# bluescarni/heyoka

Hardware: AMD Instinct MI355X
Metric: ODE systems x steps/sec (fp64) (higher is better)
Workload: dtype f64

## Files before the change

heyoka_amd/csrc/hip_emit_cluster2.cpp:

```cpp
#include <algorithm>
#include <cstdio>
#include <functional>

#include "hip_emit_cluster2_gen.hpp"
#include "logging.hpp"

namespace heyoka_amd::cluster2_detail
{

cluster2_gen::cluster2_gen(const taylor_program &p_, const emit_options &opts_, std::string &why_not_, bool allow_one_lane_,
                           std::uint32_t min_lanes_)
    : c2_emit(p_, opts_.order), p(p_), opts(opts_), why_not(why_not_), allow_one_lane(allow_one_lane_), min_lanes(min_lanes_),
      n_eq(p_.n_eq), order(opts_.order)
{
    std::string s = opts.dev.v5_opts;
    std::replace(s.begin(), s.end(), '+', ',');
    for (std::size_t b = 0, en = 0; b <= s.size(); b = en + 1u) {
        en = std::min(s.find(',', b), s.size());
        v5_flags.insert(s.substr(b, en - b));
    }
}

cluster2_attempt cluster2_gen::run()
{
// ... 1515 lines not shown
                    if (have == want && pe_lane_ev.count(cl) == 0u) {
                        pe_lane_ev[cl] = {static_cast<std::uint32_t>(ev), pe.c};
                        pe_lane_sign[cl] = pe.sign;
                        ev_on_lane[ev] = 1;
                        break;
                    }
                }
            }
        }
        const bool ev_ok = emit_event_jets_inline(*opts.ev_prog, opts, sv, ev_store, ev_code, ev_coeffs, why_ev,
                                                  use_lanes ? &hooks : nullptr, &ev_on_lane);
        if (!ev_ok) {
            pe_lane_ev.clear();
        }
        if (ev_ok) {
            ev_inline = true;
            const auto pick = [&](const std::vector<std::uint64_t> &v) {
                std::string r = std::to_string(v[0]) + "u";
                for (std::size_t c = v.size(); c-- > 1u;) {
                    r = "(l == " + std::to_string(c) + "u ? " + std::to_string(v[c]) + "u : " + r + ")";
                }
                return r;
            };
            for (std::size_t pp = 0; use_lanes && pp < hooks.leaf_vars.size(); ++pp) {
                std::vector<std::uint64_t> off, str_, zoff, zstr;
                for (const auto var : hooks.leaf_vars[pp]) {
                    const auto &lc = loc[var];
                    const auto &src_ = lc.derived ? loc[lc.parent] : lc;
                    off.push_back(src_.off);
                    str_.push_back(src_.stride);
                    zoff.push_back(lc.off);
                    zstr.push_back(lc.stride);
                }
                src << "const unsigned evo" << pp << " = " << pick(off) << " + q * " << pick(str_) << ";\n";
                if (hooks.leaf_class[pp] == 1) {
                    src << "const unsigned evz" << pp << " = " << pick(zoff) << " + q * " << pick(zstr) << ";\n";
                }
            }
            if (!pe_lane_ev.empty()) {
                std::string on = "0.0", cst = "0.0", row = std::to_string(opts.ev_prog->ev_u.size()) + "u";
                for (const auto &[lane_, evc] : pe_lane_ev) {
                    const auto ls = "(l == " + std::to_string(lane_) + "u ? ";
                    on = ls + (pe_lane_sign.at(lane_) < 0 ? "-1.0 : " : "1.0 : ") + on + ")";
                    cst = ls + fp_literal(evc.second) + " : " + cst + ")";
                    row = ls + std::to_string(evc.first) + "u : " + row + ")";
                }
                src << "const double pe_on = " << on << ";\nconst double pe_c = " << cst << ";\nconst u64 pe_row = (u64)" << row
                    << " * " << (order + 1u) << "u;\n";
            }
        }
    }
}

void cluster2_gen::text_pickup()
{
    src << R"HIP(
// Work distribution. Propagation (steps per system differ): a device-side queue, one group of systems at a time (taking
// wavefronts, which is what lets the partial-line accesses to the SoA arrays meet in L2). Single steps (equal cost per
// group): a static interleaved schedule - group = iteration * wavefronts + wavefront - with the same locality and no
const u64 hy_waves = (u64)gridDim.x * HY_WPB;
const bool hy_static = (HY_MODE != 1) && (HY_NO_STATIC == 0);
u64 hy_it = 0;
bool hy_queue_empty = false;
for (;;) {
u64 base = 0;
if (hy_static) {
    // (Exit decided per workgroup: the cooperative store of the Taylor coefficients below has workgroup barriers. A
    // wavefront beyond the end of the ensemble in a live workgroup replicates the last system, without side effects.)
    if (HY_M4 && (hy_it * (u64)gridDim.x + blockIdx.x) * (HY_WPB * SPW) >= N) break;
    base = (hy_it * hy_waves + gwave) * SPW;
    ++hy_it;
} else {
    if (lane == 0u) base = atomicAdd((u64 *)(a.counters + 2), (u64)SPW);
}
// NOTE: through readfirstlane the position is a scalar for the compiler and the exit of the work loop a wave-uniform
// branch (a shuffle / the wavefront index leave it "divergent": exec-mask bookkeeping around the whole step loop).
base = ((u64)__builtin_amdgcn_readfirstlane((unsigned)(base >> 32)) << 32) | (u64)__builtin_amdgcn_readfirstlane((unsigned)base);
if (!(HY_M4 && hy_static) && base >= N) break;
// NOTE: lanes beyond the end of the ensemble replicate the last system (no side effects).
bool live = (base + q) < N;
u64 s = live ? (base + q) : (N - 1u);
double t_hi = a.time_hi[s], t_lo = a.time_lo[s];
)HIP";
    for (std::uint32_t i = 0; i < p.n_par; ++i) {
        src << "const double par_" << i << " = a.pars[(u64)" << i << "u * N + s];\n";
    }
    for (const auto t : lane_par_tbls) {
        src << "const double lp" << t << " = a.pars[(u64)" << utname(t) << " * N + s];\n";
    }
    for_each_owner([&](auto &, auto &ow) {
        src << row0_w(ow) << " = a.state[(u64)hy_utbl[" << ow.var_tbl * L << "u + l] * N + s];\n";
    });
    src << "HY_WSYNC();\n" << (jet_lds ? "" : "__builtin_amdgcn_fence(__ATOMIC_SEQ_CST, \"wavefront\");\n");
    src << R"HIP(
hy_df tfin, rem;
tfin.hi = 0.0; tfin.lo = 0.0; rem.hi = 0.0; rem.lo = 0.0;
bool t_dir = true;
double mdt = __builtin_inf();
double step_lim = 0.0;
double thr = 0.0;
if (HY_MODE == 1) {
    tfin.hi = (a.tfin_hi != nullptr) ? a.tfin_hi[s] : a.tfin_s_hi;
    tfin.lo = (a.tfin_hi != nullptr) ? a.tfin_lo[s] : a.tfin_s_lo;
    hy_df tcur; tcur.hi = t_hi; tcur.lo = t_lo;
    rem = hy_df_sub(tfin, tcur);
    t_dir = (rem.hi > 0.0) || (rem.hi == 0.0 && rem.lo >= 0.0);
    if (a.lim != nullptr) mdt = a.lim[s];
    // (Propagation from grid point to grid point - hy_kargs::pad bit 2 in mode 1, emitted_module::grid_multi_step: the
    // system leaves the step loop after the first step which reaches a.tc_thr[s], with the coefficients of that step stored.)
    if ((a.pad & 4) != 0) thr = a.tc_thr[s];
} else {
    step_lim = a.lim[s];
    // (Taylor coefficients of a lock-step sweep on demand - hy_kargs::pad bit 2, the loop of propagate_grid() without a
    // callback: the NEXT GRID TIME of every system - a.tc_thr, or a.tfin_hi for callers of before round 6 -, and only the
    // steps which reach it store their coefficients - see emitted_module::tc_by_threshold.)
    if ((a.pad & 4) != 0) thr = (a.tc_thr != nullptr) ? a.tc_thr[s] : a.tfin_hi[s];
}
u64 n_steps = 0, iter = 0;
double min_h = __builtin_inf(), max_h = 0.0, last_h = 0.0;
i64 outcome = HY_OC_SUCCESS;
// NOTE: the step loop is left by the whole wavefront at once (wave-uniform exit): a system which has reached its final
// time keeps executing steps of length zero with all its bookkeeping frozen by selects (fin) until the other
// systems of the wavefront are done - a wavefront executes an iteration as long as one of its lanes is active
// anyway. With a per-lane exit the loop-carried values of the lanes which have left live across several
// hundred live registers of the remaining ones, which is where this toolchain's live-range splitting goes
// wrong (DESIGN.md, toolchain notes).
bool fin = false;
// (Did the system leave the step loop through a step clamped to its remaining time? hy_kargs::grid_done.)
bool gfin = false;
int nf_seen = 0;
// (Stepper with events which evaluates the event equations itself: does this system need its Taylor coefficients in
// memory? See "On-demand Taylor coefficients" below. hy_kargs::pad: bit 0 = store them for every system, bit 1 = store
// NOTHING but them - the regeneration launch on the snapshot of the state before the step.)
bool need_tc = true;
const bool hy_tc_only = HY_M4 && ((a.pad & 2) != 0);
)HIP";
    bk_lds = one_lane;
    if (bk_lds) {
        bk_store();
        src << "HY_WSYNC();\n";
    }
    src << "for (;;) {\n";
    src << body;
}

void cluster2_gen::text_selector()
{
    if (!pe_lane_ev.empty()) {
        src << "HY_WSYNC();\n";
        std::string dK[3];
        for (std::uint32_t i = 0; i < 3u; ++i) {
            src << "const double pe_d" << i << " = " << slabk(order, utname(st1.s[i][0])) << " - " << slabk(order, utname(st1.s[i][1]))
                << ";\n";
            dK[i] = "pe_d" + std::to_string(i);
        }
        for (std::uint32_t i = 0; i < 3u; ++i) {
            src << "double pe_q" << i << " = " << dK[i] << " * " << sD[i][0] << ";\n";
            for (std::uint32_t j = 1; 2u * j < order; ++j) {
                src << "pe_q" << i << " = __builtin_fma(" << sD[i][j] << ", " << sD[i][order - j] << ", pe_q" << i << ");\n";
            }
            if (order % 2u == 0u) {
                src << "pe_q" << i << " = __builtin_fma(0.5 * " << sD[i][order / 2u] << ", " << sD[i][order / 2u] << ", pe_q" << i
                    << ");\n";
            }
        }
        src << "const double pe_bh = (pe_q0 + pe_q1) + pe_q2;\n";
        pe_g.resize(order + 1u);
        src << "const double pe_b0s = " << sB[0] << " * pe_on;\n";
        src << "const double pe_g0 = pe_b0s + pe_c;\n";
        pe_g[0] = "pe_g0";
        for (std::uint32_t k = 1; k < order; ++k) {
            src << "const double pe_g" << k << " = " << sB[k] << " * pe_b0s;\n";
            pe_g[k] = "pe_g" + std::to_string(k);
        }
        src << "const double pe_g" << order << " = (pe_bh + pe_bh) * pe_on;\n";
        pe_g[order] = "pe_g" + std::to_string(order);
        src << "m0 = hy_nmax(m0, fabs(pe_g0));\nmo = hy_nmax(mo, fabs(pe_g" << order
            << "));\nmom1 = hy_nmax(mom1, fabs(pe_g" << order - 1u << "));\n";
    }

    const bool packed_tail = L >= 4u;
    const auto red_ex = [&](std::uint32_t m, const char *v) -> std::string {
        if (m == 1u) {
            return std::string("hy_dpp<0xB1>(") + v + ")";
        }
        if (m == 2u) {
            return std::string("hy_dpp<0x4E>(") + v + ")";
        }
        if (m == 4u && L % 16u == 0u) {
// ... 48 lines not shown
        for (const auto &o2 : gr.owners) {
            if (o2.derived && o2.parent == ow.col) {
                dv = &o2;
            }
        }
        tail_passes.push_back({&ow, dv, dv != nullptr && pk_tbl.count(ow.col) != 0u, {}, {}});
    });
    kstride = static_cast<std::uint64_t>(spw) * n_colp;
    if (one_lane && !m4 && jet_lds && opts.high_accuracy && packed_tail && !v5_flag("notailrd")) {
        src << "// (Jet reads of the final evaluation issued ahead of the selector.)\n";
        const auto hoist = [&](const std::string &ex) {
            auto nm = "trd" + std::to_string(n_trd++);
            src << "const double " << nm << " = " << ex << ";\n";
            return nm;
        };
        for (auto &tp : tail_passes) {
            const auto cs = std::to_string(tp.ow->col);
            if (tp.packed) {
                const auto &tb = pk_tbl.at(tp.ow->col);
                if (!lane_sum) {
                    src << "const double *const pk_jh" << cs << " = jetw + q * " << jet_sys(*tp.ow) << "u + hy_utbl[" << tb[1] * L << "u + l];\n";
                    src << "const double *const pk_fh" << cs << " = lds_fac + hy_utbl[" << tb[2] * L << "u + l];\n";
                }
                tp.rows.resize(order + 1u);
                tp.facs.resize(order + 1u);
                for (std::uint32_t k = 1; k <= order; ++k) {
                    tp.rows[k] = hoist("pk_jh" + cs + "[" + std::to_string((k - 1u) * kstride) + "]");
                    tp.facs[k] = hoist("pk_fh" + cs + "[" + std::to_string(k) + "]");
                }
            } else {
                for (std::uint32_t k = 0; k <= order; ++k) {
                    tp.rows.push_back(hoist("jr" + cs + "[" + std::to_string(k * kstride) + "]"));
                }
            }
        }
        src << "__builtin_amdgcn_sched_barrier(0);\n";
    }
    if (packed_tail) {
        src << "const double nw = (hy_q0 & (nv <= 1.0)) ? 1.0 : nv;\n";
        src << "const double lg = " << (sel_scalar ? "hy_sel_log_s" : "hy_sel_log") << "(nw);\n";
        src << "const double lg0 = hy_dpp<0x00>(lg), lg1 = hy_dpp<0x55>(lg), lg2 = hy_dpp<0xAA>(lg);\n";
        src << "const double lr_o = (lg0 - lg1) * " << fp_literal(1. / static_cast<double>(order)) << ";\n";
        src << "const double lr_om1 = (lg0 - lg2) * " << fp_literal(1. / static_cast<double>(order - 1u)) << ";\n";
        src << "const double rho_m = " << (sel_scalar ? "hy_sel_exp_s" : "exp") << "(hy_min(lr_o, lr_om1));\n";
    } else {
        src << "const double num_rho = (m0 <= 1.0) ? 1.0 : m0;\n";
        src << "const double lr_o = log(num_rho / mo) * " << fp_literal(1. / static_cast<double>(order)) << ";\n";
        src << "const double lr_om1 = log(num_rho / mom1) * " << fp_literal(1. / static_cast<double>(order - 1u)) << ";\n";
        src << "const double rho_m = exp(hy_min(lr_o, lr_om1));\n";
    }
    if (bk_lds) {
        bk_load();
    }
    src << R"HIP(
double lim;
if (HY_MODE == 1) {
    hy_df m; m.lo = 0.0;
    // NOTE: selects, not an if/else on the (per-lane) direction: see the note on HY_LIBM1.
    m.hi = t_dir ? mdt : -mdt;
    const bool lt_fwd = hy_df_lt(rem, m), lt_bwd = hy_df_lt(m, rem);
    const bool rem_first = (t_dir & lt_fwd) | (!t_dir & lt_bwd);
    lim = rem_first ? rem.hi : m.hi;
} else {
    lim = step_lim;
}
lim = fin ? 0.0 : lim;
)HIP";
    src << "double h = rho_m * " << fp_literal(rhofac(order)) << ";\n";
    src << "h = hy_min(h, fabs(lim));\nh = (lim < 0.0) ? -h : h;\n";
    src << "h = fin ? 0.0 : h;\n";
}

void cluster2_gen::text_event_exclusion()
{
    if (ev_inline) {
        src << "bool maybe0 = false, pe_m0 = false;\n{\nconst double ah = fabs(h);\n";
        for (const auto &c : ev_coeffs) {
            if (c.empty()) {
                continue;
            }
            src << "{\ndouble r = fabs(" << c[order] << ");\n";
            for (std::uint32_t k = order - 1u; k >= 1u; --k) {
                src << "r = r * ah + fabs(" << c[k] << ");\n";
            }
            src << "r = r * ah;\nmaybe0 = maybe0 | !(fabs(" << c[0] << ") > r * 1.00000001);\n}\n";
        }
        if (!pe_g.empty()) {
            src << "{\ndouble r = fabs(" << pe_g[order] << ");\n";
            for (std::uint32_t k = order - 1u; k >= 1u; --k) {
                src << "r = r * ah + fabs(" << pe_g[k] << ");\n";
            }
            src << "r = r * ah;\npe_m0 = (pe_on != 0.0) & !(fabs(" << pe_g[0] << ") > r * 1.00000001);\n}\n";
        }
        src << "}\nneed_tc = ((a.pad & 1) != 0);\nbool ev_possible = false;\n";
        const auto sys_any = [&](const char *v) {
            return "(((__builtin_amdgcn_ballot_w64(" + std::string(v) + ") >> ((threadIdx.x & 63u) & " + std::to_string(64u - L) + "u)) & "
                   + std::to_string((std::uint64_t(1) << L) - 1u) + "ull) != 0ull)";
        };
        src << "if (__builtin_amdgcn_ballot_w64(maybe0 | pe_m0) != 0ull) {\n";
        src << "bool maybe = false, maybe_te = false;\nconst double lo_h = (h < 0.0) ? h : 0.0, hi_h = (h < 0.0) ? 0.0 : h;\n";
        const auto enclosure = [&](const std::vector<std::string> &c) {
            src << "{\ndouble lo = " << c[order] << ", hi = lo, mm = fabs(lo);\n";
            for (std::uint32_t i = 1; i <= order; ++i) {
                src << "{\nconst double p0 = lo * lo_h, p1 = lo * hi_h, p2 = hi * lo_h, p3 = hi * hi_h;\n"
                    << "const double mn = fmin(fmin(p0, p1), fmin(p2, p3)), mx = fmax(fmax(p0, p1), fmax(p2, p3));\n"
                    << "lo = mn + " << c[order - i] << ";\nhi = mx + " << c[order - i] << ";\n"
                    << "mm = fmax(mm, fmax(fabs(lo), fabs(hi)));\n}\n";
            }
        };
        for (std::size_t ci = 0; ci < ev_coeffs.size(); ++ci) {
            const auto &c = ev_coeffs[ci];
            if (c.empty()) {
                continue;
            }
            enclosure(c);
            src << "const bool excl = (((lo > 0.0) & (hi > 0.0)) | ((lo < 0.0) & (hi < 0.0))) & (fmin(fabs(lo), fabs(hi)) > 1e-8 * mm);\n"
                << "maybe = maybe | !excl;\n" << (ci < opts.n_t_events ? "maybe_te = maybe_te | !excl;\n" : "") << "}\n";
        }
        src << "bool pe_m = false;\n";
        if (!pe_g.empty()) {
// ... 103 lines not shown
                    }
                }
            }
        }
        src << xn << " = res;\n";
        if (dv != nullptr) {
            src << xd << " = resd;\n";
        }
        src << "}\n";
        const auto new_at = [&](const owner_slot &o) {
            return ev_inline ? ("slab[" + std::to_string(o.col * L) + "u + l]") : row0_w(o);
        };
        upd.emplace_back(xn, row0_r(ow), new_at(ow));
        if (dv != nullptr) {
            upd.emplace_back(xd, row0_r(*dv), new_at(*dv));
        }
    }
    if (n_trd_used != n_trd) {
        throw std::logic_error("hy_taylor (one lane per pair): " + std::to_string(n_trd - n_trd_used)
                               + " jet reads of the final evaluation were issued ahead of the selector and not consumed");
    }
    for (std::uint32_t c = 0; !one_lane && c < n_hslots; ++c) {
        upd.emplace_back("xn" + std::to_string(c), "hc" + std::to_string(c) + "[0]", "hc" + std::to_string(c) + "[0]");
        if (m4) {
            src << "const double xn" << c << " = hc" << c << "[0];\n";
            continue;
        }
        src << "double xn" << c << ";\n{\nconst double *c = hc" << c << ";\n";
        if (opts.high_accuracy) {
            src << "double res = c[0], comp = 0.0, cur_h = h;\n#pragma unroll\n";
            src << "for (unsigned k = 1; k <= " << order << "u; ++k) {\n";
            src << "const double tmp = c[(u64)k * " << kstride << "u] * cur_h;\nconst double y = tmp - comp;\n";
            src << "const double t = res + y;\ncomp = (t - res) - y;\nres = t;\ncur_h = cur_h * h;\n}\n";
        } else {
            src << "double res = c[(u64)" << order << "u * " << kstride << "u];\n#pragma unroll\n";
            src << "for (unsigned k = 1; k <= " << order << "u; ++k) {\n";
            src << "res = c[(u64)(" << order << "u - k) * " << kstride << "u] + res * h;\n}\n";
        }
        src << "xn" << c << " = res;\n}\n";
    }
    src << R"HIP(
double nt_hi, nt_lo;
{
    hy_df tcur; tcur.hi = t_hi; tcur.lo = t_lo;
    hy_df hh; hh.hi = h; hh.lo = 0.0;
    const hy_df nt = hy_df_add(tcur, hh);
    nt_hi = nt.hi; nt_lo = nt.lo;
}
int nfi = !(hy_finite(nt_hi) && hy_finite(nt_lo)) ? 1 : 0;
)HIP";
    for (const auto &u3 : upd) {
        src << "nfi |= !hy_finite(" << std::get<0>(u3) << ") ? 1 : 0;\n";
    }
    src << "{\nconst u64 nfb = __builtin_amdgcn_ballot_w64(nfi != 0);\n";
    if (L == 64u) {
        src << "nfi = (nfb != 0ull) ? 1 : 0;\n}\n";
    } else {
        src << "nfi = (((nfb >> ((threadIdx.x & 63u) & " << (64u - L) << "u)) & " << ((std::uint64_t(1) << L) - 1u)
            << "ull) != 0ull) ? 1 : 0;\n}\n";
    }
    if (one_lane && jet_lds && !m4) {
        src << "const bool hy_reach = (h > 0.0) ? (nt_hi >= thr) : (nt_hi <= thr);\n";
        src << "const bool tc_sys = ((a.pad & 4) == 0) | (!fin & ((h == 0.0) | (h == lim) | hy_reach));\n";
        src << "if (a.tc != nullptr && tc_sys) {\n";
    } else {
        src << (jet_lds ? "if (a.tc != nullptr && !HY_M4) {\n" : "if (a.tc != nullptr) {\n");
    }
    for_each_owner([&](auto &, auto &ow) {
        if (ow.derived) {
            src << "{\nconst double *c = jr" << ow.parent << ";\ndouble *tcp = a.tc + ((u64)hy_utbl[" << ow.var_tbl * L
                << "u + l] * " << (order + 1u) << "u) * N + s;\n*tcp = " << row0_r(ow) << ";\ntcp += N;\n"
                << "#pragma nounroll\nfor (unsigned k = 1; k <= " << order << "u; ++k) {\n*tcp = c[(u64)(k - 1u) * "
                << kstride << "u] * hy_rk[k];\ntcp += N;\n}\n}\n";
            return;
        }
        src << "{\nconst double *c = jr" << ow.col << ";\ndouble *tcp = a.tc + ((u64)hy_utbl[" << ow.var_tbl * L
            << "u + l] * " << (order + 1u) << "u) * N + s;\n"
            << "#pragma nounroll\nfor (unsigned k = 0; k <= " << order << "u; ++k) {\n*tcp = c[(u64)k * "
            << kstride << "u];\ntcp += N;\n}\n}\n";
    });
    src << "}\n";
    src << "HY_WSYNC();\n" << jet_fence;
    for (const auto &u3 : upd) {
        src << std::get<2>(u3) << " = (fin | nostate) ? " << std::get<1>(u3) << " : " << std::get<0>(u3) << ";\n";
    }
    src << "HY_WSYNC();\n" << jet_fence;
    src << R"HIP(
{
    // Bookkeeping of the reference's step() / propagate_until() loops (src/taylor_adaptive_batch.cpp:632-727,
    // :1395-1520) on values frozen once the system is done.
    const bool nf = nfi != 0;
    const i64 oc_new = nf ? HY_OC_ERR_NF_STATE : ((h == lim) ? HY_OC_TIME_LIMIT : HY_OC_SUCCESS);
    bool done = nf | (HY_MODE != 1);
    const u64 ns_new = n_steps + ((!done & (h != 0.0)) ? 1u : 0u);
    const bool upd = !done & (oc_new == HY_OC_SUCCESS);
    const double ah = fabs(h);
    const double mn_new = upd ? hy_min(min_h, ah) : min_h;
    const double mx_new = upd ? hy_max(max_h, ah) : max_h;
    done |= (h == rem.hi);
    gfin = fin ? gfin : (h == rem.hi);
    done |= HY_GRID_STOP;
    hy_df tnew; tnew.hi = nt_hi; tnew.lo = nt_lo;
    const hy_df rem_new = hy_df_sub(tfin, tnew);
    const u64 it_new = iter + 1u;
    const bool sl = !done & (it_new == a.max_steps);
    const i64 oc_fin = sl ? HY_OC_STEP_LIMIT : oc_new;
    done |= sl;
    nf_seen |= (!fin & nf & !nostate) ? 1 : 0;
    // (fin: h = 0, hence nt = t, rem_new = rem, ns_new = n_steps, no min / max update - see above.)
    t_hi = notime ? t_hi : nt_hi;
    t_lo = notime ? t_lo : nt_lo;
    last_h = fin ? last_h : h;
    outcome = fin ? outcome : oc_fin;
    n_steps = ns_new;
    min_h = mn_new;
    max_h = mx_new;
    rem.hi = rem_new.hi;
    rem.lo = rem_new.lo;
    iter = it_new;
    fin = fin | done;
}
)HIP";
}

void cluster2_gen::text_refill_and_tail()
{
    const bool refill = one_lane && !m4 && jet_lds && p.n_par == 0u && lane_par_tbls.empty() && L < 64u
                        && opts.dev.refill;
    if (refill) {
        src << "if (!hy_static && !hy_queue_empty && __builtin_amdgcn_ballot_w64(fin) != 0ull) {\n";
        for_each_owner([&](auto &, auto &ow) {
            src << "if (fin && ovalid" << ow.col << " && live) a.state[(u64)hy_utbl[" << ow.var_tbl * L
                << "u + l] * N + s] = " << row0_w(ow) << ";\n";
        });
        src << R"HIP(
if (fin && l == 0u && live) {
    a.time_hi[s] = t_hi;
    a.time_lo[s] = t_lo;
    a.last_h[s] = last_h;
    a.outcome[s] = outcome;
    a.min_h[s] = min_h;
    a.max_h[s] = max_h;
    a.n_steps[s] = n_steps;
    if (HY_GRID_FLAGS) a.grid_done[s] = gfin ? 1.0 : 0.0;
    if (nf_seen != 0) atomicAdd(a.counters, 1u);
}
// 2. The next system of the queue, for every finished system of the wavefront (its lane 0 asks, the others listen).
u64 snew = 0;
if (fin && l == 0u) snew = atomicAdd((u64 *)(a.counters + 2), (u64)1);
{
    const int src_lane = (int)((threadIdx.x & 63u) - l);
    const unsigned lo_ = (unsigned)__shfl((int)(unsigned)snew, src_lane, 64);
    const unsigned hi_ = (unsigned)__shfl((int)(unsigned)(snew >> 32), src_lane, 64);
    snew = ((u64)hi_ << 32) | (u64)lo_;
}
const bool got = fin && (snew < N);
// (The queue position only grows: one request beyond the end means that the queue is empty - stop asking.)
if (__builtin_amdgcn_ballot_w64(fin && !got) != 0ull) hy_queue_empty = true;
live = fin ? got : live;
nf_seen = fin ? 0 : nf_seen;
s = got ? snew : s;
// 3. Its state, times and limits; a fresh set of counters.
if (got) {
    t_hi = a.time_hi[s];
    t_lo = a.time_lo[s];
)HIP";
        for_each_owner([&](auto &, auto &ow) {
            src << row0_w(ow) << " = a.state[(u64)hy_utbl[" << ow.var_tbl * L << "u + l] * N + s];\n";
        });
        src << R"HIP(
    tfin.hi = (a.tfin_hi != nullptr) ? a.tfin_hi[s] : a.tfin_s_hi;
    tfin.lo = (a.tfin_hi != nullptr) ? a.tfin_lo[s] : a.tfin_s_lo;
    hy_df tcur; tcur.hi = t_hi; tcur.lo = t_lo;
    rem = hy_df_sub(tfin, tcur);
    t_dir = (rem.hi > 0.0) || (rem.hi == 0.0 && rem.lo >= 0.0);
    mdt = (a.lim != nullptr) ? a.lim[s] : __builtin_inf();
    thr = ((a.pad & 4) != 0) ? a.tc_thr[s] : 0.0;
    n_steps = 0;
    iter = 0;
    min_h = __builtin_inf();
    max_h = 0.0;
    last_h = 0.0;
    outcome = HY_OC_SUCCESS;
    fin = false;
    gfin = false;
}
HY_WSYNC();
)HIP";
        if (bk_lds) {
            bk_store(2);
        }
        src << "}\n";
    }
    if (bk_lds) {
        bk_store(1);
    }
    src << R"HIP(
if (__builtin_amdgcn_ballot_w64(!fin) == 0ull) break;
}
if (nf_seen != 0 && l == 0u && live) atomicAdd(a.counters, 1u);
)HIP";
    if (jet_lds && m4) {
        const auto spb = wpb * spw;
        src << "{\nconst int hy_wg_tc = __syncthreads_or(need_tc ? 1 : 0);\n";
        src << "if (hy_wg_tc == 0 && threadIdx.x == 0u) atomicAdd(a.counters + 4, 1u);\n";
        src << "if (hy_wg_tc != 0) {\n";
        src << "const u64 bs0 = base - (u64)wib * SPW;\n";
        src << "for (unsigned idx = threadIdx.x; idx < " << n_tc_rows * spb << "u; idx += " << bs << "u) {\n";
        src << "const unsigned sy = idx % " << spb << "u;\nconst unsigned long long te = lds_tcsrc[idx / " << spb << "u];\n";
        src << "const unsigned row = (unsigned)(te & 0xfffffull), off = (unsigned)((te >> 20) & 0xfffffull), sst = "
               "(unsigned)(te >> 40);\n";
        src << "const u64 sg = bs0 + sy;\n";
        src << "const double val = lds_jet[(sy / SPW) * " << jet_doubles_per_wave << "u + off + (sy % SPW) * sst];\n";
        src << "if (sg < N) a.tc[(u64)row * N + sg] = val;\n}\n}\n__syncthreads();\n}\n";
    }
    src << R"HIP(
)HIP";
    for_each_owner([&](auto &, auto &ow) {
        if (m4 && !ev_inline) {
            return;
        }
        src << "if (ovalid" << ow.col << " && live && !hy_tc_only) a.state[(u64)hy_utbl[" << ow.var_tbl * L << "u + l] * N + s] = "
            << (ev_inline ? ("slab[" + std::to_string(ow.col * L) + "u + l]") : row0_w(ow)) << ";\n";
    });
    src << R"HIP(
if (l == 0u && live && !hy_tc_only) {
    if (!HY_M4) {
        if (HY_MODE != 2) {
            a.time_hi[s] = t_hi;
            a.time_lo[s] = t_lo;
        } else {
            const_cast<double *>(a.lim)[s] = last_h;
        }
    }
    if (!HY_M4 || HY_EV_INLINE) a.last_h[s] = last_h;
    a.outcome[s] = outcome;
    if (HY_MODE == 1) {
        a.min_h[s] = min_h;
        a.max_h[s] = max_h;
        a.n_steps[s] = n_steps;
        if (HY_GRID_FLAGS) a.grid_done[s] = gfin ? 1.0 : 0.0;
    }
}
}
}
)HIP";
}

void cluster2_gen::finish()
{
    res.mod.source = src.str();
    res.mod.kernel_name = "hy_taylor";
    res.mod.dout_name = "hy_dout";
    res.mod.block_size = bs;
    res.mod.lanes_per_system = L;
    res.mod.lds_bytes = 0;
    res.mod.mode = emit_mode::cluster;
    res.mod.n_statements = e.n_stmt;
    res.mod.scratch_per_wave = jet_lds ? 0u : jet_doubles_per_wave;
    res.mod.persistent = true;
    if (pairk) {
        res.mod.compile_flags = "-mllvm -disable-machine-licm";
        if (one_lane) {
            res.mod.compile_flags += " -Xclang -target-feature -Xclang -load-store-opt -mllvm -amdgpu-load-store-vectorizer=0";
        }
    }
    res.mod.tc_optional = true;
    res.mod.cluster_mode4 = m4;
    res.mod.events_in_stepper = ev_inline;
    res.mod.compact_tc = compact_tc;
    res.mod.tc_by_threshold = one_lane && jet_lds && !m4;
    res.mod.grid_multi_step = res.mod.tc_by_threshold;
    res.jets_in_lds = one_lane && jet_lds;
    res.variant = variant;
    res.mod.cluster_generation = one_lane ? 5 : (pair_split ? 3 : 2);
    res.mod.notes = std::string(one_lane ? "cluster mode v5 (one lane per pair, 2 wavefronts per SIMD): "
                                     : (pair_split ? "cluster mode v3 (lane pairs, 2 wavefronts per SIMD): " : "cluster mode v2 (pipelined): "))
                + std::to_string(nc) + " clusters of " + std::to_string(t0().size())
                + " nodes, L=" + std::to_string(L) + ", " + std::to_string(pl.n_slots) + " LDS slots x2, "
                + std::to_string(n_own) + " state-variable owner slots, " + std::to_string(utbl.size())
                + " slot tables, jets in " + (jet_lds ? "LDS" : "global scratch")
                + (one_lane ? ", slab layout: " + std::to_string(bank_cost) + " conflict cycles per step in the model" : std::string{})
                + (lane_sum ? ", later sums reduced across the lanes of the first round" : "")
                + (ev_inline ? "; event equations, final step size and state update inside the stepper" : "");
}

}
namespace heyoka_amd
{

emitted_module emit_cluster_v2(const taylor_program &p, const emit_options &opts, std::string &why_not)
{
    std::string why1;
    const bool try_one_lane = opts.cluster_kernel == 0 || opts.cluster_kernel == 5;
    for (const std::uint32_t min_lanes : {4u, 8u, 16u}) {
        why1.clear();
        auto at = cluster2_detail::cluster2_gen(p, opts, why1, try_one_lane, min_lanes).run();
        const bool is_v5 = why1.empty() && at.variant == cluster2_detail::cluster2_variant::one_lane, in_lds = at.jets_in_lds;
        if (try_one_lane) {
            detail::log_message(log_level::debug, "one-lane-per-pair kernel, at least " + std::to_string(min_lanes) + " lanes per system: "
                                              + (!why1.empty() ? why1 : (!is_v5 ? "not applicable" : (in_lds ? "accepted" : "the jets of the systems of a CU do not fit in its LDS"))));
        }
        if (why1.empty() && (in_lds || !is_v5)) {
            why_not.clear();
            return std::move(at.mod);
        }
        if (!try_one_lane || (!why1.empty() && !at.more_lanes_cure) || (why1.empty() && !is_v5)) {
            break;
        }
    }
    return cluster2_detail::cluster2_gen(p, opts, why_not, false, 4u).run().mod;
}

}
```

heyoka_amd/csrc/hip_emit_cluster2_gen.hpp:

```cpp
#pragma once

#include <array>
#include <map>
#include <set>
#include <tuple>

#include "hip_emit_cluster_plan.hpp"
#include "hip_emit_detail.hpp"

namespace heyoka_amd::cluster2_detail
{

using cluster_detail::cluster_plan;
using cluster_detail::is_var;
using emit_detail::prelude;
using emit_detail::rhofac;
using emit_detail::ssa_emitter;
using psel = ssa_emitter::part_sel;

enum class cluster2_variant { pipelined, lane_pair, one_lane };

struct cluster2_attempt {
    emitted_module mod;
    cluster2_variant variant = cluster2_variant::pipelined;
    bool jets_in_lds = false;
    bool more_lanes_cure = false;
};

struct c2_variant {
    cluster2_variant variant = cluster2_variant::pipelined;
    bool one_lane = false, pair_split = false;
    bool pairk = false;
    bool m4 = false;
    bool frx = false;
    bool fuse_rx = false;
    bool frx_regs = false, merged = false;
    bool lane_sum = false;
    std::set<std::string> v5_flags;
    bool v5_flag(const char *name) const { return v5_flags.count(name) != 0u; }
};

struct c2_geometry {
    cluster_plan pl;
    cluster_detail::pair_pattern pp;
    std::vector<char> cu;
    std::uint32_t nc = 0, L = 0, spw = 0, bs = 0, wpb = 0, n_ext = 0, n_out = 0, n_cst = 0;
    const std::vector<std::uint32_t> &t0() const { return pl.clusters[0]; }
    std::array<std::uint32_t, 3> body_vars(std::uint32_t c, std::uint32_t sd) const
    {
        return {pl.ext_u[c][pp.de[0][sd]], pl.ext_u[c][pp.de[1][sd]], pl.ext_u[c][pp.de[2][sd]]};
    }
};

struct owner_slot {
    std::size_t out_tbl = 0;
    std::size_t var_tbl = 0;
    std::uint32_t col = 0;
    std::uint32_t cbase = 0;
    std::uint32_t n_valid = 0;
    std::vector<std::string> xname;
    bool slab_needed = true;
    bool derived = false;
    std::uint32_t parent = 0;
    bool mapped = false, reduced = false;
    std::size_t col_tbl = 0;
    std::uint32_t valid_mask = 0;
};
struct glue_round {
    std::vector<std::size_t> arg_tbl;
    std::size_t out_tbl = 0;
    std::uint32_t n_valid = 0;
    bool exported = true;
    std::vector<owner_slot> owners;
    std::vector<std::string> par_name;
    std::vector<std::string> c0name;
    std::vector<std::size_t> coef_tbl;
    bool reduced = false;
};

struct c2_layout {
    std::map<std::uint32_t, std::vector<std::uint32_t>> att;
    std::vector<std::uint32_t> grp_natt;
    std::vector<char> rx_fused;
    std::vector<std::uint32_t> rx_src;
    std::vector<char> glue_read;
    std::vector<std::uint32_t> lane_pr, lane_rx;
    bool wide_rd = false;
    bool vexch = false;
    std::vector<std::array<std::uint32_t, 2>> vx_col;
    std::vector<std::array<std::uint32_t, 3>> wide_pr, wide_rx;
    std::uint32_t slab_stride_opt = 0;
    std::uint64_t bank_cost = 0;
// ... 80 lines not shown

    cluster2_gen(const taylor_program &p, const emit_options &opts, std::string &why_not, bool allow_one_lane, std::uint32_t min_lanes);
    cluster2_attempt run();

    void plan_and_select_variant(), anchors_and_reaction_fusion(), layout_one_lane(), lds_layout_and_lane_tables(),
        build_glue_rounds(), layout_jets_and_schedule(), init_order_programs(), emit_step_body(),
        text_helpers_and_constant_tables(), text_kernel_prologue(), text_event_equations(), text_pickup(), text_selector(),
        text_event_exclusion(), text_final_evaluation_and_update(), text_refill_and_tail(), finish();
    void number_glue_slots(std::uint32_t ns), place_wide_read_slots(), plan_lane_sums(std::uint32_t n_first), renumber_sv_slots();
    std::uint32_t n_rounds_of(std::size_t g) const;
    std::pair<std::uint32_t, bool> round_node(std::size_t g, std::uint32_t r, std::uint32_t l) const;
    template <typename F>
    void for_each_owner(F &&f)
    {
        for (auto &rg : rounds) {
            for (auto &gr : rg) {
                for (auto &ow : gr.owners) {
                    f(gr, ow);
                }
            }
        }
    }

    std::size_t add_utbl(std::vector<std::uint32_t> v, bool is_slot = true);
    std::size_t add_dtbl(std::vector<double> v);
    std::string utname(std::size_t t) const { return utexpr[t]; }
    std::string dtname(std::size_t t) const { return one_lane ? ("dtl[" + std::to_string(t * L) + "]") : ("dt" + std::to_string(t)); }
    std::string coefname(std::size_t t) const { return frx_regs ? ("frc" + std::to_string(t)) : dtname(t); }
    std::uint32_t pr_slot(std::uint32_t pr_u, std::uint32_t rx_u, std::uint32_t dflt) const;
    std::string lane_par(std::vector<std::uint32_t> idx);
    std::uint64_t jet_off(const owner_slot &ow) const { return vexch ? ow.cbase : static_cast<std::uint64_t>(spw) * ow.cbase; }
    std::uint32_t jet_sys(const owner_slot &ow) const { return vexch ? (ow.derived ? n_dcol : n_col) : ow.n_valid; }
    bool pack_tail_slot(const owner_slot &ow, const owner_slot *dv) const;
    std::string slabk(std::uint32_t k, const std::string &tbl) const;
    std::string jet_at(std::uint32_t k, std::uint32_t col) const
    {
        return "jc" + std::to_string(col) + "[" + std::to_string(static_cast<std::uint64_t>(k) * spw * n_colp) + "]";
    }
    void sync() { os << "HY_WSYNC();\n"; }
    void sched_fence() { os << "__builtin_amdgcn_sched_barrier(0);\n"; }
    std::string row0_r(const owner_slot &ow) const { return (ow.derived ? "x0r" : "jr") + std::to_string(ow.col) + "[0]"; }
    std::string row0_w(const owner_slot &ow) const { return (ow.derived ? "x0c" : "jc") + std::to_string(ow.col) + "[0]"; }
    void publish_sv(owner_slot &ow, std::uint32_t k, const std::string &name);
    std::string wide_read(const std::string &tbl);
    std::vector<std::string> emit_glue_reads(std::size_t g, std::uint32_t r, std::uint32_t k), emit_pair_reads(std::uint32_t k),
        emit_single_reads(std::uint32_t k);
    void emit_glue_compute(std::size_t g, std::uint32_t r, std::uint32_t k, const std::vector<std::string> &names),
        emit_pair_compute(std::uint32_t k, const std::vector<std::string> &rdv);
    void emit_glue_round(std::size_t g, std::uint32_t r, std::uint32_t k) { emit_glue_compute(g, r, k, emit_glue_reads(g, r, k)); }
    void emit_pair_order(std::uint32_t k) { emit_pair_compute(k, emit_pair_reads(k)); }
    void emit_store(const std::string &stmt) { os << stmt; }
    void emit_single_compute(std::uint32_t k, const std::vector<std::string> &rdv), emit_single_history(std::uint32_t k), emit_cluster(std::uint32_t k);
    void bk_store(int which = 0), bk_load();
    std::string tail_val(const std::vector<std::string> &names, std::uint32_t k, const std::string &ex);
};

}
```

heyoka_amd/csrc/hip_emit_cluster2_orders.cpp:

```cpp
#include <cstdio>

#include "hip_emit_cluster2_gen.hpp"

namespace heyoka_amd::cluster2_detail
{

std::string cluster2_gen::slabk(std::uint32_t k, const std::string &tbl) const
{
    return (k % 2u == 0u || buf_stride == 0u) ? ("slab[" + tbl + "]")
                                              : ("slab[" + tbl + " + " + std::to_string(buf_stride) + "u]");
}

void cluster2_gen::publish_sv(owner_slot &ow, std::uint32_t k, const std::string &name)
{
    ow.xname[k] = name;
    if (ow.slab_needed) {
        os << slabk(k, utname(ow.out_tbl)) << " = " << name << ";\n";
    }
    if (k != 0u && !ow.derived) {
        os << jet_at(k, ow.col) << " = " << name << ";\n";
    }
    const char *acc = (k == 0u) ? "m0" : (k == order ? "mo" : (k == order - 1u ? "mom1" : nullptr));
    if (acc != nullptr && ow.reduced && k != 0u) {
        os << acc << " = hy_nmax(" << acc << ", fabs(ovalid" << ow.col << " ? " << name << " : 0.0));\n";
// ... 368 lines not shown
                } else {
                    hm[i] = e.def(ssa_emitter::mul(sD[i][K / 2u], sD[i][K / 2u]));
                }
            }
        }
        if (K % 2u == 0u) {
            for (std::uint32_t i = 0; i < (merged_sq ? 1u : 3u); ++i) {
                hq[i] = hq[i].empty() ? e.def(ssa_emitter::mul("0.5", hm[i]))
                                      : e.def("__builtin_fma(0.5, " + hm[i] + ", " + hq[i] + ")");
            }
        }
        const auto t1 = e.def(ssa_emitter::mul(fp_literal(-(pp.ex + 1.) / static_cast<double>(K)), hU));
        pow_pre = e.def("__builtin_fma(" + fp_literal(pp.ex) + ", " + hT + ", " + t1 + ")");
    } else {
        pow_pre.clear();
    }
}

void cluster2_gen::emit_cluster(std::uint32_t k)
{
    if (pair_split) {
        emit_pair_order(k);
        return;
    }
    for (std::uint32_t part = 1; part < n_parts; ++part) {
        e.emit_partials(t0_ids, k, part, n_parts);
    }
    for (std::uint32_t x = 0; x < n_ext; ++x) {
        if (ext_const[x] != 0 && k > 0u) {
            e.val(pl.ext_u[0][x], k) = "0.0";
            continue;
        }
        e.val(pl.ext_u[0][x], k) = e.def(slabk(k, utname(ext_tbl[x])));
    }
    if (overlap) {
        sched_fence();
        e.emit_partials_sel(t0_ids, k + 1u, psel::early_b);
        if (fence2) {
            sched_fence();
        }
    }
    for (const auto u : t0()) {
        e.node_finish(u - n_eq, k);
    }
    for (std::uint32_t x = 0; x < n_out; ++x) {
        os << slabk(k, utname(out_tbl[x])) << " = " << e.val(t0()[pl.out_pos[x]], k) << ";\n";
    }
}

void cluster2_gen::bk_store(int which)
{
    std::uint32_t f = 0;
    for (const auto *nm : bk_fields_d) {
        const std::string n_ = nm;
        const bool constant = n_ == "tfin.hi" || n_ == "tfin.lo" || n_ == "mdt" || n_ == "step_lim" || n_ == "thr";
        if (which == 0 || (which == 1) != constant) {
            src << "bk[" << f << "] = " << nm << ";\n";
        }
        ++f;
    }
    if (which == 2) {
        return;
    }
    src << "bk[" << f++ << "] = __longlong_as_double((long long)n_steps);\n";
    src << "bk[" << f++ << "] = __longlong_as_double((long long)iter);\n";
    src << "bk[" << f++ << "] = __longlong_as_double((long long)outcome);\n";
    src << "bk[" << f++ << "] = __longlong_as_double((long long)((t_dir ? 1 : 0) | (nf_seen != 0 ? 2 : 0) | (gfin ? 4 : 0)));\n";
}

void cluster2_gen::bk_load()
{
    std::uint32_t f = 0;
    for (const auto *nm : bk_fields_d) {
        src << nm << " = bk[" << f++ << "];\n";
    }
    src << "n_steps = (u64)__double_as_longlong(bk[" << f++ << "]);\n";
    src << "iter = (u64)__double_as_longlong(bk[" << f++ << "]);\n";
    src << "outcome = (i64)__double_as_longlong(bk[" << f++ << "]);\n";
    src << "{\nconst long long fl = __double_as_longlong(bk[" << f++ << "]);\nt_dir = (fl & 1) != 0;\nnf_seen = (fl & 2) != 0 ? 1 : 0;\ngfin = (fl & 4) != 0;\n}\n";
}

std::string cluster2_gen::tail_val(const std::vector<std::string> &names, std::uint32_t k, const std::string &ex)
{
    if (names.empty()) {
        return ex;
    }
    ++n_trd_used;
    return names.at(k);
}

}
```

Before: 827.9 million.

## Add plain-step fast path skipping per-step bookkeeping in one-lane stepper

Adds a 'plain step' path for one-lane propagation. When the whole wavefront can take the Taylor-selected step size, a conservative lower bound of the remaining time (rlb) shows the step is far from the final time, no limit applies and all values are finite. In that case the kernel skips the double-float remaining-time subtraction, the clamping, the non-finite ballot and the full bookkeeping selects, and it stores fewer bookkeeping fields to LDS. Otherwise it falls back to the ordinary path, recomputing the remaining time there. The trade-off is more code and branching, extra register pressure, and a new A/B benchmarking script.

```diff
diff --git a/heyoka_amd/csrc/hip_emit_cluster2.cpp b/heyoka_amd/csrc/hip_emit_cluster2.cpp
--- a/heyoka_amd/csrc/hip_emit_cluster2.cpp
+++ b/heyoka_amd/csrc/hip_emit_cluster2.cpp
@@ -1591,9 +1591,24 @@
     }
 }
 
+namespace
+{
+
+std::string exchanged(std::string text, const std::string &from, const std::string &to)
+{
+    const auto pos = text.find(from);
+    if (pos == std::string::npos || text.find(from, pos + 1u) != std::string::npos) {
+        throw std::logic_error("hy_taylor (one lane per pair): the plain-step text does not find exactly one '" + from + "'");
+    }
+    return text.replace(pos, from.size(), to);
+}
+
+}
+
 void cluster2_gen::text_pickup()
 {
-    src << R"HIP(
+    plain_step = one_lane && !m4 && jet_lds && !v5_flag("noplainstep");
+    std::string work = R"HIP(
 // Work distribution. Propagation (steps per system differ): a device-side queue, one group of systems at a time (taking
 // wavefronts, which is what lets the partial-line accesses to the SoA arrays meet in L2). Single steps (equal cost per
 // group): a static interleaved schedule - group = iteration * wavefronts + wavefront - with the same locality and no
@@ -1621,6 +1636,12 @@
 u64 s = live ? (base + q) : (N - 1u);
 double t_hi = a.time_hi[s], t_lo = a.time_lo[s];
 )HIP";
+    if (plain_step) {
+        work = exchanged(work, "const u64 hy_waves = ", "const u64 hy_gwave = (u64)blockIdx.x * HY_WPB + (u64)__builtin_amdgcn_readfirstlane(threadIdx.x >> 6);\n"
+                                                         "const u64 hy_waves = ");
+        work = exchanged(work, "hy_waves + gwave) * SPW;", "hy_waves + hy_gwave) * SPW;");
+    }
+    src << work;
     for (std::uint32_t i = 0; i < p.n_par; ++i) {
         src << "const double par_" << i << " = a.pars[(u64)" << i << "u * N + s];\n";
     }
@@ -1631,7 +1652,7 @@
         src << row0_w(ow) << " = a.state[(u64)hy_utbl[" << ow.var_tbl * L << "u + l] * N + s];\n";
     });
     src << "HY_WSYNC();\n" << (jet_lds ? "" : "__builtin_amdgcn_fence(__ATOMIC_SEQ_CST, \"wavefront\");\n");
-    src << R"HIP(
+    std::string pickup = R"HIP(
 hy_df tfin, rem;
 tfin.hi = 0.0; tfin.lo = 0.0; rem.hi = 0.0; rem.lo = 0.0;
 bool t_dir = true;
@@ -1674,6 +1695,13 @@
 bool need_tc = true;
 const bool hy_tc_only = HY_M4 && ((a.pad & 2) != 0);
 )HIP";
+    if (plain_step) {
+        pickup = exchanged(pickup, "hy_df tfin, rem;\ntfin.hi = 0.0; tfin.lo = 0.0; rem.hi = 0.0; rem.lo = 0.0;\n",
+                           "hy_df tfin;\ntfin.hi = 0.0; tfin.lo = 0.0;\n// (A lower bound of the magnitude of the remaining time: see the plain step.)\n"
+                           "double rlb = 0.0;\n");
+        pickup = exchanged(pickup, "    rem = hy_df_sub(tfin, tcur);\n", "    const hy_df rem = hy_df_sub(tfin, tcur);\n");
+    }
+    src << pickup;
     bk_lds = one_lane;
     if (bk_lds) {
         bk_store();
@@ -1828,7 +1856,7 @@
     if (bk_lds) {
         bk_load();
     }
-    src << R"HIP(
+    const std::string limit = R"HIP(
 double lim;
 if (HY_MODE == 1) {
     hy_df m; m.lo = 0.0;
@@ -1842,6 +1870,25 @@
 }
 lim = fin ? 0.0 : lim;
 )HIP";
+    if (plain_step) {
+        src << "#define HY_PLAIN_STEP ((HY_MODE == 1) & ((a.pad & 4) == 0) & (a.tc == nullptr))\n";
+        src << "const double h_sel = rho_m * " << fp_literal(rhofac(order)) << ";\n";
+        src << "const double h_two = h_sel + h_sel;\n";
+        src << "const bool pl_no = fin | !((h_sel > 0.0) & (h_two <= rlb) & (h_two <= mdt)) | (iter + 1u == a.max_steps);\n";
+        src << "double h;\nbool at_lim = false, at_rem = false;\n";
+        src << "if (HY_PLAIN_STEP && __builtin_amdgcn_ballot_w64(pl_no) == 0ull) {\n"
+               "h = t_dir ? h_sel : -h_sel;\n"
+               "rlb = __builtin_fma(-0x1p-100, fabs(t_hi) + h_sel, (rlb - h_sel) * 0x1.ffffffffffff8p-1);\n} else {\n"
+               "hy_df rem; rem.hi = 0.0; rem.lo = 0.0;\n";
+        src << exchanged(limit, "double lim;\nif (HY_MODE == 1) {\n",
+                         "double lim;\nif (HY_MODE == 1) {\n    hy_df tcur; tcur.hi = t_hi; tcur.lo = t_lo;\n    rem = hy_df_sub(tfin, tcur);\n");
+        src << "h = hy_min(h_sel, fabs(lim));\nh = (lim < 0.0) ? -h : h;\nh = fin ? 0.0 : h;\n";
+        src << "at_lim = (h == lim);\nat_rem = (h == rem.hi);\n";
+        src << "rlb = __builtin_fma(-0x1p-100, fabs(t_hi) + fabs(h), (hy_min(t_dir ? rem.hi : -rem.hi, 0x1p+1000) * 0x1.ffffffffffff8p-1 - fabs(h))"
+               " * 0x1.ffffffffffff8p-1);\n}\n";
+        return;
+    }
+    src << limit;
     src << "double h = rho_m * " << fp_literal(rhofac(order)) << ";\n";
     src << "h = hy_min(h, fabs(lim));\nh = (lim < 0.0) ? -h : h;\n";
     src << "h = fin ? 0.0 : h;\n";
@@ -2051,16 +2098,21 @@
     for (const auto &u3 : upd) {
         src << "nfi |= !hy_finite(" << std::get<0>(u3) << ") ? 1 : 0;\n";
     }
-    src << "{\nconst u64 nfb = __builtin_amdgcn_ballot_w64(nfi != 0);\n";
-    if (L == 64u) {
-        src << "nfi = (nfb != 0ull) ? 1 : 0;\n}\n";
-    } else {
-        src << "nfi = (((nfb >> ((threadIdx.x & 63u) & " << (64u - L) << "u)) & " << ((std::uint64_t(1) << L) - 1u)
-            << "ull) != 0ull) ? 1 : 0;\n}\n";
+    const auto nf_of_the_system = [&]() {
+        src << "{\nconst u64 nfb = __builtin_amdgcn_ballot_w64(nfi != 0);\n";
+        if (L == 64u) {
+            src << "nfi = (nfb != 0ull) ? 1 : 0;\n}\n";
+        } else {
+            src << "nfi = (((nfb >> ((threadIdx.x & 63u) & " << (64u - L) << "u)) & " << ((std::uint64_t(1) << L) - 1u)
+                << "ull) != 0ull) ? 1 : 0;\n}\n";
+        }
+    };
+    if (!plain_step) {
+        nf_of_the_system();
     }
     if (one_lane && jet_lds && !m4) {
         src << "const bool hy_reach = (h > 0.0) ? (nt_hi >= thr) : (nt_hi <= thr);\n";
-        src << "const bool tc_sys = ((a.pad & 4) == 0) | (!fin & ((h == 0.0) | (h == lim) | hy_reach));\n";
+        src << "const bool tc_sys = ((a.pad & 4) == 0) | (!fin & ((h == 0.0) | " << (plain_step ? "at_lim" : "(h == lim)") << " | hy_reach));\n";
         src << "if (a.tc != nullptr && tc_sys) {\n";
     } else {
         src << (jet_lds ? "if (a.tc != nullptr && !HY_M4) {\n" : "if (a.tc != nullptr) {\n");
@@ -2080,11 +2132,34 @@
     });
     src << "}\n";
     src << "HY_WSYNC();\n" << jet_fence;
+    if (plain_step) {
+        src << "if (HY_PLAIN_STEP && __builtin_amdgcn_ballot_w64(pl_no | (nfi != 0)) == 0ull) {\n";
+        for (const auto &u3 : upd) {
+            src << std::get<2>(u3) << " = " << std::get<0>(u3) << ";\n";
+        }
+        src << "HY_WSYNC();\n" << jet_fence;
+        src << R"HIP(
+{
+    const double ah = fabs(h);
+    t_hi = nt_hi;
+    t_lo = nt_lo;
+    last_h = h;
+    outcome = HY_OC_SUCCESS;
+    n_steps = n_steps + 1u;
+    iter = iter + 1u;
+    min_h = hy_min(min_h, ah);
+    max_h = hy_max(max_h, ah);
+}
+)HIP";
+        bk_store(3);
+        src << "} else {\n";
+        nf_of_the_system();
+    }
     for (const auto &u3 : upd) {
         src << std::get<2>(u3) << " = (fin | nostate) ? " << std::get<1>(u3) << " : " << std::get<0>(u3) << ";\n";
     }
     src << "HY_WSYNC();\n" << jet_fence;
-    src << R"HIP(
+    std::string ordinary = R"HIP(
 {
     // Bookkeeping of the reference's step() / propagate_until() loops (src/taylor_adaptive_batch.cpp:632-727,
     // :1395-1520) on values frozen once the system is done.
@@ -2120,6 +2195,14 @@
     fin = fin | done;
 }
 )HIP";
+    if (plain_step) {
+        ordinary = exchanged(ordinary, "    hy_df tnew; tnew.hi = nt_hi; tnew.lo = nt_lo;\n    const hy_df rem_new = hy_df_sub(tfin, tnew);\n", "");
+        ordinary = exchanged(ordinary, "hence nt = t, rem_new = rem, ns_new", "hence nt = t, ns_new");
+        ordinary = exchanged(ordinary, "    rem.hi = rem_new.hi;\n    rem.lo = rem_new.lo;\n", "");
+        ordinary = exchanged(ordinary, "((h == lim) ? HY_OC_TIME_LIMIT", "(at_lim ? HY_OC_TIME_LIMIT");
+        ordinary = exchanged(ordinary, "    done |= (h == rem.hi);\n    gfin = fin ? gfin : (h == rem.hi);\n", "    done |= at_rem;\n    gfin = fin ? gfin : at_rem;\n");
+    }
+    src << ordinary;
 }
 
 void cluster2_gen::text_refill_and_tail()
@@ -2167,7 +2250,7 @@
         for_each_owner([&](auto &, auto &ow) {
             src << row0_w(ow) << " = a.state[(u64)hy_utbl[" << ow.var_tbl * L << "u + l] * N + s];\n";
         });
-        src << R"HIP(
+        std::string fresh = R"HIP(
     tfin.hi = (a.tfin_hi != nullptr) ? a.tfin_hi[s] : a.tfin_s_hi;
     tfin.lo = (a.tfin_hi != nullptr) ? a.tfin_lo[s] : a.tfin_s_lo;
     hy_df tcur; tcur.hi = t_hi; tcur.lo = t_lo;
@@ -2186,6 +2269,10 @@
 }
 HY_WSYNC();
 )HIP";
+        if (plain_step) {
+            fresh = exchanged(fresh, "    rem = hy_df_sub(tfin, tcur);\n", "    const hy_df rem = hy_df_sub(tfin, tcur);\n    rlb = 0.0;\n");
+        }
+        src << fresh;
         if (bk_lds) {
             bk_store(2);
         }
@@ -2193,6 +2280,9 @@
     }
     if (bk_lds) {
         bk_store(1);
+    }
+    if (plain_step) {
+        src << "}\n";
     }
     src << R"HIP(
 if (__builtin_amdgcn_ballot_w64(!fin) == 0ull) break;
@@ -2281,6 +2371,7 @@
                 + " slot tables, jets in " + (jet_lds ? "LDS" : "global scratch")
                 + (one_lane ? ", slab layout: " + std::to_string(bank_cost) + " conflict cycles per step in the model" : std::string{})
                 + (lane_sum ? ", later sums reduced across the lanes of the first round" : "")
+                + (plain_step ? ", plain steps leave out the bookkeeping of the step loop" : "")
                 + (ev_inline ? "; event equations, final step size and state update inside the stepper" : "");
 }
 
diff --git a/heyoka_amd/csrc/hip_emit_cluster2_gen.hpp b/heyoka_amd/csrc/hip_emit_cluster2_gen.hpp
--- a/heyoka_amd/csrc/hip_emit_cluster2_gen.hpp
+++ b/heyoka_amd/csrc/hip_emit_cluster2_gen.hpp
@@ -38,6 +38,7 @@
     bool lane_sum = false;
     std::set<std::string> v5_flags;
     bool v5_flag(const char *name) const { return v5_flags.count(name) != 0u; }
+    bool plain_step = false;
 };
 
 struct c2_geometry {
@@ -224,6 +225,7 @@
     void emit_store(const std::string &stmt) { os << stmt; }
     void emit_single_compute(std::uint32_t k, const std::vector<std::string> &rdv), emit_single_history(std::uint32_t k), emit_cluster(std::uint32_t k);
     void bk_store(int which = 0), bk_load();
+    std::string bk_field(const char *nm) const;
     std::string tail_val(const std::vector<std::string> &names, std::uint32_t k, const std::string &ex);
 };
 
diff --git a/heyoka_amd/csrc/hip_emit_cluster2_orders.cpp b/heyoka_amd/csrc/hip_emit_cluster2_orders.cpp
--- a/heyoka_amd/csrc/hip_emit_cluster2_orders.cpp
+++ b/heyoka_amd/csrc/hip_emit_cluster2_orders.cpp
@@ -444,10 +444,10 @@
 {
     std::uint32_t f = 0;
     for (const auto *nm : bk_fields_d) {
-        const std::string n_ = nm;
+        const std::string n_ = bk_field(nm);
         const bool constant = n_ == "tfin.hi" || n_ == "tfin.lo" || n_ == "mdt" || n_ == "step_lim" || n_ == "thr";
-        if (which == 0 || (which == 1) != constant) {
-            src << "bk[" << f << "] = " << nm << ";\n";
+        if (!n_.empty() && (which == 0 || ((which == 1 || which == 3) != constant))) {
+            src << "bk[" << f << "] = " << n_ << ";\n";
         }
         ++f;
     }
@@ -457,14 +457,29 @@
     src << "bk[" << f++ << "] = __longlong_as_double((long long)n_steps);\n";
     src << "bk[" << f++ << "] = __longlong_as_double((long long)iter);\n";
     src << "bk[" << f++ << "] = __longlong_as_double((long long)outcome);\n";
+    if (which == 3) {
+        return;
+    }
     src << "bk[" << f++ << "] = __longlong_as_double((long long)((t_dir ? 1 : 0) | (nf_seen != 0 ? 2 : 0) | (gfin ? 4 : 0)));\n";
+}
+
+std::string cluster2_gen::bk_field(const char *nm) const
+{
+    const std::string n_ = nm;
+    if (plain_step && n_ == "rem.hi") {
+        return "rlb";
+    }
+    return (plain_step && n_ == "rem.lo") ? std::string{} : n_;
 }
 
 void cluster2_gen::bk_load()
 {
     std::uint32_t f = 0;
     for (const auto *nm : bk_fields_d) {
-        src << nm << " = bk[" << f++ << "];\n";
+        if (const auto n_ = bk_field(nm); !n_.empty()) {
+            src << n_ << " = bk[" << f << "];\n";
+        }
+        ++f;
     }
     src << "n_steps = (u64)__double_as_longlong(bk[" << f++ << "]);\n";
     src << "iter = (u64)__double_as_longlong(bk[" << f++ << "]);\n";
diff --git a/profiles/experiments/ab_trees.py b/profiles/experiments/ab_trees.py
--- /dev/null
+++ b/profiles/experiments/ab_trees.py
@@ -0,0 +1,126 @@
+#!/usr/bin/env python
+import glob
+import json
+import os
+import shutil
+import statistics
+import subprocess
+import sys
+import tempfile
+
+HERE = os.path.dirname(os.path.abspath(__file__))
+sys.path.insert(0, os.path.dirname(HERE))
+import summarize_rocprof
+
+BENCH = ["--gpus", "1", "--steps", "20", "--warmup", "5"]
+PROFILED = ["--workload", "outer_ss", "--no-cpu-baseline", "--no-extra-workloads", "--steps", "4", "--warmup", "1"]
+PASSES = (("SQ_INSTS_VALU", "SQ_INSTS_LDS", "SQ_WAVE_CYCLES"), ("SQ_ACTIVE_INST_VALU", "SQ_WAIT_ANY", "SQ_WAVE_CYCLES"))
+
+
+class Log:
+    def __init__(self, path):
+        self.f = open(path, "a")
+
+    def __call__(self, text=""):
+        print(text, flush=True)
+        self.f.write(text + "\n")
+        self.f.flush()
+
+
+def child(cmd, tree, limit):
+    env = {k: v for k, v in os.environ.items() if k not in ("HEYOKA_AMD_V5_OPTS", "PYTHONPATH")}
+    r = subprocess.run(["timeout", "-k", "10", str(limit)] + cmd, cwd=tree, env=env, capture_output=True, text=True)
+    if r.returncode != 0:
+        sys.exit("ab_trees: %s in %s ended with status %d; stopping here.\n%s" % (" ".join(cmd), tree, r.returncode, r.stderr[-3000:]))
+    return r.stdout
+
+
+def bench_line(out):
+    lines = [ln for ln in out.split("\n") if ln.startswith("{")]
+    return lines[-1], json.loads(lines[-1])
+
+
+def bench(trees, log, runs):
+    log("# bench.py %s, parent and new in alternation (parent first), one session (the lines as printed, cut to 400 characters)" % " ".join(BENCH))
+    vals = {"parent": [], "new": []}
+    for _ in range(runs):
+        for tag in ("parent", "new"):
+            line, b = bench_line(child([sys.executable, "bench.py"] + BENCH, trees[tag], 400))
+            vals[tag].append(float(b["value"]))
+            log("%s %s" % (tag, line[:400]))
+    log()
+    mean = {t: statistics.mean(v) for t, v in vals.items()}
+    sd = {t: statistics.stdev(v) for t, v in vals.items()}
+    for t in ("parent", "new"):
+        log("%-7s n = %d, mean = %.6e, sample standard deviation = %.3e (%.3f %%)" % (t + ":", len(vals[t]), mean[t], sd[t], 100.0 * sd[t] / mean[t]))
+    d = mean["new"] - mean["parent"]
+    log("new mean - parent mean = %.3e = %.1f parent standard deviations (asked: more than 10); ratio new / parent = %.4f"
+        % (d, d / sd["parent"], mean["new"] / mean["parent"]))
+    lo, hi = min(vals["new"]), max(vals["parent"])
+    log("smallest new value %.6e %s largest parent value %.6e" % (lo, ">" if lo > hi else "<=", hi))
+    log("bar met: %s" % ("yes" if d > 10.0 * sd["parent"] and lo > hi else "NO"))
+
+
+def profiled(tree, args, limit=400):
+    d = tempfile.mkdtemp(prefix="ab_trees_")
+    child(["rocprofv3"] + args + ["-d", d, "-o", "p", "--", sys.executable, os.path.join(tree, "bench.py")] + PROFILED, tree, limit)
+    dbs = glob.glob(os.path.join(d, "**", "*.db"), recursive=True)
+    if not dbs:
+        sys.exit("ab_trees: rocprofv3 left no database in " + d)
+    return d, dbs[0]
+
+
+def trace(trees, log):
+    log("# rocprofv3 --kernel-trace --stats of bench.py %s, one run each" % " ".join(PROFILED))
+    avg = {}
+    for tag in ("parent", "new"):
+        d, db = profiled(trees[tag], ["--kernel-trace", "--stats"])
+        txt, _ = summarize_rocprof.kernel_stats(db)
+        for ln in txt.split("\n"):
+            if ln.startswith("hy_taylor") or ln.startswith("kernel "):
+                log("%s: %s" % (tag, ln))
+            if "timed launches" in ln:
+                avg[tag] = float(ln.split("avg_ns = ")[1])
+        shutil.rmtree(d, ignore_errors=True)
+    log("timed launches: kernel time new / parent = %.4f, i.e. rate x %.4f" % (avg["new"] / avg["parent"], avg["parent"] / avg["new"]))
+
+
+def pmc(trees, log):
+    log("# rocprofv3 --pmc (two passes of their own per tree, no tracing domains), last hy_taylor dispatch of bench.py %s" % " ".join(PROFILED))
+    got = {}
+    for tag in ("parent", "new"):
+        got[tag] = {}
+        for names in PASSES:
+            d, db = profiled(trees[tag], ["--pmc"] + list(names))
+            rows = summarize_rocprof.counters(db)
+            last = max(r[0] for r in rows)
+            for r in rows:
+                if r[0] == last:
+                    got[tag][r[1]] = float(r[2])
+                    got[tag]["kernel_ms"] = r[10] / 1e6
+            shutil.rmtree(d, ignore_errors=True)
+        log("%s: kernel %.2f ms" % (tag, got[tag]["kernel_ms"]))
+        for k in sorted(got[tag]):
+            if k != "kernel_ms":
+                log("  %-24s %16.0f  %.3f of SQ_WAVE_CYCLES" % (k, got[tag][k], got[tag][k] / got[tag]["SQ_WAVE_CYCLES"]))
+    log()
+    for k in sorted(got["new"]):
+        if k != "kernel_ms":
+            log("%-22s new / parent = %.4f" % (k, got["new"][k] / got["parent"][k]))
+
+
+def main():
+    if len(sys.argv) < 5 or sys.argv[1] not in ("bench", "trace", "pmc"):
+        sys.exit(__doc__)
+    trees = {"parent": os.path.abspath(sys.argv[2]), "new": os.path.abspath(sys.argv[3])}
+    log = Log(sys.argv[4])
+    if sys.argv[1] == "bench":
+        bench(trees, log, int(sys.argv[sys.argv.index("--runs") + 1]) if "--runs" in sys.argv else 5)
+    elif sys.argv[1] == "trace":
+        trace(trees, log)
+    else:
+        pmc(trees, log)
+
+
+if __name__ == "__main__":
+    main()
```

New measurement: 843.2 million (median of 6 runs). 1.8% higher.
